# ProjectTorreyPines/TorJ.jl

Hardware: AMD Instinct MI355X
Metric: ray-steps/sec, 1e5-ray EC fan on 1 MI355X (+ 2/4/8-GPU scaling) (higher is better)
Workload: dtype f64

## Files before the change

torj.jl_amd/csrc/torj_args.hpp:

```cpp
#pragma once
#include "torj_math.hpp"

struct TraceArgs {
    const double *coef;
    const double *cellp;
    Grid g;
    Consts k;
    double omega;
    int mode;
    double ds;
    int n_steps;
    int chunk_steps;
    double psi_exit;
    double P_min;
    int n;
    const double *x0;
    const double *N0;
    const double *w;
    double *state;
    int *status;
    int *steps;
    int n_psi;
    const double *grid;
    double *dP;
// ... 36 lines not shown

struct SplitArgs {
    double *ain;
    double *alpha;
    unsigned *awork;
    double *psib;
    double *cbx;
    double *tx;
    int *tinfo;
    double *stau, *spsi, *sPdep;
    int *sinfo;
    unsigned char *zflag;
    double zval;
    int k0, kb;
    int nf;
    int tile_cap;
    double tile_margin;
    int traj_mode;
    int nan_step;
    unsigned long long *defer;
    unsigned *defer_cnt;
    int defer_lrm;
    int zlatch;
};

constexpr int kSplitMaxSteps = 1 << 24;
__device__ __forceinline__ int info_steps(int v) { return v & 0xffffff; }
__device__ __forceinline__ int info_status(int v) { return (unsigned)v >> 24; }
__device__ __forceinline__ int make_info(int steps, int st) { return steps | (st << 24); }

#ifndef TORJ_AIN_TRAJ_MATH
#define TORJ_AIN_TRAJ_MATH 0
#endif
#ifndef TORJ_TRAJ_WAVES
#define TORJ_TRAJ_WAVES TORJ_MIN_WAVES
#endif
#ifndef TORJ_ALPHA_WAVES
#define TORJ_ALPHA_WAVES 6
#endif
#ifndef TORJ_ALPHA_UNROLL
#define TORJ_ALPHA_UNROLL 1
#endif
#ifndef TORJ_TILE_NODES
#define TORJ_TILE_NODES 256
#endif
constexpr int kTileNodes = TORJ_TILE_NODES;
// ... 28 lines not shown
```

torj.jl_amd/csrc/torj_fitdepo.hpp:

```cpp
#pragma once
#include "torj_math.hpp"

namespace torj {

constexpr int kSmpBlk = 64;
TORJ_HD size_t smp_at(size_t j, int i, size_t rows) {
    return ((size_t)((unsigned)i / kSmpBlk) * rows + j) * kSmpBlk + (unsigned)i % kSmpBlk;
}
TORJ_HD size_t smp_elems(size_t n, size_t rows) { return (n + kSmpBlk - 1) / kSmpBlk * kSmpBlk * rows; }

struct FitArgs {
    const double *coef;
    Grid g;
    int n, n_psi;
    double ds;
    const double *grid;
    const double *w;
    const double *x_launch;
    const double *s0;
    const int *steps;
    const double *smp_psi, *smp_dpds, *smp_s;
    size_t rows;
    int s_uniform;
    double *E, *Gpsi, *GP;
    int *cnt;
    double *Fopen;
    double *dPs;
    int *kstar;
    double *dP;
    double *Pray;
    const int *npts;
};

TORJ_HD int imin(int x, int y) { return x < y ? x : y; }
TORJ_HD int imax(int x, int y) { return x > y ? x : y; }

constexpr int kChunk = 8;
constexpr int kWalkChunk = 4;
constexpr int kWalkChunkStream = 1;

struct RayData {
    const FitArgs *a;
    int i, m;
    double s0, psiL;
    TORJ_HD double S(int j) const {
        if (a->npts) return a->smp_s[smp_at(j, i, a->rows)];
        if (j == 0) return 0.0;
        return a->s_uniform ? fma((double)(j - 1), a->ds, s0) : a->smp_s[smp_at(j - 1, i, a->rows)];
    }
    TORJ_HD double h(int j) const { return (j == 0 && !a->npts) ? s0 : S(j + 1) - S(j); }
    TORJ_HD double Ypsi(int j) const {
        if (a->npts) return a->smp_psi[smp_at(j, i, a->rows)];
        return j == 0 ? psiL : a->smp_psi[smp_at(j - 1, i, a->rows)];
    }
// ... 553 lines not shown
```

torj.jl_amd/csrc/torj_hip.hip:

```cpp
#include <hip/hip_runtime.h>

#include <algorithm>
#include <cmath>
#include <cstring>
#include <mutex>
#include <vector>

#include "../../include/torj_hip.h"
#include "torj_math.hpp"
#include "torj_entry.hpp"
#include "torj_fitdepo.hpp"
#include "torj_warm.hpp"

using namespace torj;

#include "torj_host_util.hpp"
#include "torj_args.hpp"
#include "torj_k_fused.hpp"
#include "torj_k_traj.hpp"
#include "torj_k_alpha.hpp"
#include "torj_k_scan.hpp"
#include "torj_k_depo.hpp"
#include "torj_k_points.hpp"
#include "torj_k_beams.hpp"
// ... 136 lines not shown
        if (p->stage.h_pinned)
            (void)hipHostFree(p->stage.h);
        else
            free(p->stage.h);
    }
    for (int r = 0; r < 2; r++) {
        if (p->stage.up[r]) (void)hipEventDestroy(p->stage.up[r]);
        if (p->stage.tr[r]) (void)hipEventDestroy(p->stage.tr[r]);
        if (p->stage.dn[r]) (void)hipEventDestroy(p->stage.dn[r]);
    }
    if (p->stage.sc) (void)hipStreamDestroy(p->stage.sc);
    if (p->d_coef) (void)hipFree(p->d_coef);
    if (p->d_cellp) (void)hipFree(p->d_cellp);
    if (p->stream) (void)hipStreamDestroy(p->stream);
    if (p->ev_Nin) (void)hipEventDestroy(p->ev_Nin);
    if (p->ev_Nout) (void)hipEventDestroy(p->ev_Nout);
    if (p->sched.d) (void)hipFree(p->sched.d);
    if (p->fit.d) (void)hipFree(p->fit.d);
    if (p->d_flags) (void)hipFree(p->d_flags);
    if (p->chunk.d) (void)hipFree(p->chunk.d);
    for (hipEvent_t e : p->ev_pool) (void)hipEventDestroy(e);
    if (p->ws.d) (void)hipFree(p->ws.d);
    if (p->beams.d) (void)hipFree(p->beams.d);
    if (p->split.d) (void)hipFree(p->split.d);
    if (p->batch.d) (void)hipFree(p->batch.d);
    for (int q = 0; q < torj_plasma_s::kRing; q++) {
        if (p->ev_T[q]) (void)hipEventDestroy(p->ev_T[q]);
        if (p->ev_A[q]) (void)hipEventDestroy(p->ev_A[q]);
        if (p->ev_S[q]) (void)hipEventDestroy(p->ev_S[q]);
    }
    if (p->ev_J) (void)hipEventDestroy(p->ev_J);
    if (p->ev_F) (void)hipEventDestroy(p->ev_F);
    if (p->ev_D) (void)hipEventDestroy(p->ev_D);
    if (p->stream2) (void)hipStreamDestroy(p->stream2);
    if (p->streamT) (void)hipStreamDestroy(p->streamT);
    if (p->streamS) (void)hipStreamDestroy(p->streamS);
    if (p->streamD) (void)hipStreamDestroy(p->streamD);
    delete p;
    return 0;
}

int torj_plasma_get_coefs(torj_plasma_t p, int field, double *out) {
    if (!p || field < 0 || field > 5) return fail("bad plasma handle or field index");
    const size_t nodes = (size_t)(p->g.nR + 2) * (p->g.nZ + 2);
    for (size_t k = 0; k < nodes; k++) out[k] = p->coef[k * kNF + kFieldSlot[field]];
    return 0;
// ... 761 lines not shown
```

torj.jl_amd/csrc/torj_k_beams.hpp:

```cpp
#pragma once
#include "torj_args.hpp"
#include "torj_entry.hpp"
#include "torj_k_depo.hpp"
#include "torj_k_fused.hpp"
#include "torj_k_points.hpp"

__device__ __forceinline__ int beam_of(const BeamRec *beams, int n_beams, int i) {
    int lo = 0, hi = n_beams - 1;
    while (lo < hi) {
        const int mid = (lo + hi) >> 1;
        if (beams[mid].hi > i)
            hi = mid;
        else
            lo = mid + 1;
    }
    return lo;
}

__device__ __forceinline__ TraceArgs beam_args(const BeamsArgs &ba, int b, const BeamRec &br) {
    TraceArgs a = ba.a;
    a.omega = br.omega, a.k = br.k, a.mode = br.mode;
    if (a.dP) a.dP += (size_t)b * (size_t)(a.n_psi + 1);
    return a;
}

template <int ABS, int DEPO, bool TRAJ, int LPR = 1>
__global__ void __launch_bounds__(64, TORJ_MIN_WAVES) k_trace_beams(BeamsArgs ba) {
    const BeamWave wv = ba.waves[blockIdx.x];
    const BeamRec br = ba.beams[wv.beam];
    const TraceArgs a = beam_args(ba, wv.beam, br);
    const int i = wv.first + (int)threadIdx.x / LPR, sub = (int)threadIdx.x % LPR;
    AlbajarWork work = {};
    unsigned long long steps = 0;
    if (i < br.hi) {
        RayState r;
        load_start(a, i, r);
        const double w = (DEPO == kDepoBinned && a.w) ? a.w[i] : 1.0;
        ray_segment<ABS, DEPO, TRAJ, LPR>(a, i, w, r, a.n_steps, work, sub);
        if (sub == 0) {
            store_state(a, i, r);
// ... 2 lines not shown
        }
    }
    flush_counters(a, steps, 4ull * steps, work);
}

template <int ABS>
__global__ void __launch_bounds__(64) k_final_alpha_beams(BeamsArgs ba) {
    const TraceArgs &a = ba.a;
    const int i = blockIdx.x * 64 + threadIdx.x;
    if (i >= a.n) return;
    const int k = a.steps[i];
    if (k <= 0) return;
    const BeamRec br = ba.beams[beam_of(ba.beams, ba.n_beams, i)];
    double x[3], N[3], du[6], al = 0.0;
#pragma unroll
    for (int c = 0; c < 3; c++) {
        x[c] = a.state[c * a.n + i];
        N[c] = a.state[(3 + c) * a.n + i];
    }
    if constexpr (ABS != 0) ray_rhs_m<ABS>(a.coef, a.g, br.k, c_gl, br.omega, br.mode, a.abs_model, x, N, du, al, nullptr);
    a.smp_dpds[smp_at(k, i, a.smp_rows)] = exp(-a.state[6 * a.n + i]) * al;
}

__global__ void __launch_bounds__(256) k_shell_sum_beams(FitArgs a, const BeamRec *beams) {
    const int k = blockIdx.x;
    const int lo = beams[blockIdx.y].lo, nb = beams[blockIdx.y].hi - lo;
    double acc = 0.0;
    constexpr int kB = 8;
    const bool shell = k < a.n_psi - 1;
    const double *row = (shell ? a.dPs + (size_t)k * a.n : a.Pray) + lo;
    const double *wr = a.w ? a.w + lo : nullptr;
    const int *kstar = a.kstar + lo;
    for (int i0 = threadIdx.x; i0 < nb; i0 += 256 * kB) {
        double v[kB], wv[kB];
        bool on[kB];
#pragma unroll
        for (int u = 0; u < kB; u++) {
            const int i = i0 + 256 * u;
            on[u] = i < nb;
            v[u] = on[u] ? row[i] : 0.0;
            wv[u] = on[u] && wr ? wr[i] : 1.0;
            if (shell && on[u]) on[u] = k > kstar[i];
        }
#pragma unroll
        for (int u = 0; u < kB; u++)
            if (on[u]) acc += wv[u] * v[u];
    }
    __shared__ double red[4];
// ... 29 lines not shown
```

torj.jl_amd/csrc/torj_k_depo.hpp:

```cpp
#pragma once
#include "torj_args.hpp"
#include "torj_fitdepo.hpp"

constexpr int kFitGridLds = 4096;

__global__ void __launch_bounds__(64, 2) k_fit_depo(FitArgs a) {
    extern __shared__ double s_grid[];
    if (a.n_psi <= kFitGridLds) {
        for (int k = threadIdx.x; k < a.n_psi; k += 64) s_grid[k] = a.grid[k];
        __syncthreads();
        a.grid = s_grid;
    }
    const int i = blockIdx.x * 64 + threadIdx.x;
    if (i >= a.n) return;
    const double xl[3] = {a.x_launch[i], a.x_launch[a.n + i], a.x_launch[2 * a.n + i]};
    fit_depo_ray<kOpenCache>(a, i, psi_at(a.coef, a.g, xl));
}
__device__ __forceinline__ bool fit_grid_lds(FitArgs &a) {
    extern __shared__ double s_grid[];
    if (a.n_psi > kFitGridLds) return false;
    for (int k = threadIdx.x; k < a.n_psi; k += 64) s_grid[k] = a.grid[k];
    __syncthreads();
    a.grid = s_grid;
    return true;
}
__device__ __forceinline__ bool depo_stream_gate(const FitArgs &a, const DepoStream &ds, const int *sinfo,
                                                 int s_cap, int i, int &S, double &psiL) {
    const int v = __hip_atomic_load(sinfo + i, __ATOMIC_RELAXED, __HIP_MEMORY_SCOPE_AGENT);
    if (info_status(v) != ST_OK) return false;
    S = min(info_steps(v), s_cap);
    const int j = ds.v[kDsJ * (size_t)a.n + i];
    if ((j < 0 ? 0 : j) + kDepoQ + 3 + kDepoW > S) return false;
    psiL = 0.0;
    if (j < 0) {
        const double xl[3] = {a.x_launch[i], a.x_launch[a.n + i], a.x_launch[2 * a.n + i]};
        psiL = psi_at(a.coef, a.g, xl);
    }
    return true;
}
// ... 11 lines not shown
__global__ void __launch_bounds__(64, TORJ_DEPO_ELIM_WAVES) k_depo_elim(FitArgs a, DepoStream ds, const int *sinfo,
                                                                        int s_cap) {
    const int i = blockIdx.x * 64 + threadIdx.x;
    int S;
    double psiL;
    if (i >= a.n || !depo_stream_gate(a, ds, sinfo, s_cap, i, S, psiL)) return;
    fit_depo_stream_elim(a, ds, i, psiL, S);
}
#ifndef TORJ_DEPO_WALK_WAVES
#define TORJ_DEPO_WALK_WAVES 3
#endif
__global__ void __launch_bounds__(64, TORJ_DEPO_WALK_WAVES) k_depo_walk(FitArgs a, DepoStream ds, const int *sinfo,
                                                                        int s_cap) {
    fit_grid_lds(a);
    const int i = blockIdx.x * 64 + threadIdx.x;
    int S;
    double psiL;
    if (i >= a.n || !depo_stream_gate(a, ds, sinfo, s_cap, i, S, psiL)) return;
    fit_depo_stream_walk(a, ds, i, psiL, S);
}
__global__ void __launch_bounds__(64, 2) k_depo_tail(FitArgs a, DepoStream ds) {
    fit_grid_lds(a);
    const int i = blockIdx.x * 64 + threadIdx.x;
    if (i >= a.n) return;
    const double xl[3] = {a.x_launch[i], a.x_launch[a.n + i], a.x_launch[2 * a.n + i]};
    fit_depo_tail(a, ds, i, psi_at(a.coef, a.g, xl));
}
__global__ void __launch_bounds__(64) k_profile_samples(FitArgs a, const long *off, const double *s,
                                                        const double *x, size_t n_all, const double *dpds) {
    const int i = blockIdx.x * 64 + threadIdx.x;
    if (i >= a.n) return;
    for (int j = 0; j < a.npts[i]; j++) {
        const size_t q = (size_t)off[i] + j;
        const double xq[3] = {x[q], x[n_all + q], x[2 * n_all + q]};
        const size_t o = smp_at(j, i, a.rows);
        const_cast<double *>(a.smp_psi)[o] = psi_at(a.coef, a.g, xq);
        const_cast<double *>(a.smp_dpds)[o] = dpds[q];
        const_cast<double *>(a.smp_s)[o] = s[q];
    }
}
__global__ void __launch_bounds__(64, 2) k_fit_profile(FitArgs a) {
    extern __shared__ double s_grid[];
    if (a.n_psi <= kFitGridLds) {
        for (int k = threadIdx.x; k < a.n_psi; k += 64) s_grid[k] = a.grid[k];
        __syncthreads();
        a.grid = s_grid;
    }
    const int i = blockIdx.x * 64 + threadIdx.x;
    if (i >= a.n) return;
    fit_depo_ray<kOpenCache>(a, i, 0.0);
}
__global__ void __launch_bounds__(256) k_grid_check(const double *grid, int n, int *flags) {
    bool bad = false;
    for (int k = threadIdx.x + 1; k < n; k += 256) bad |= !(grid[k] > grid[k - 1]);
    if (bad) atomicOr(flags, 1);
}

__global__ void __launch_bounds__(256) k_shell_sum(FitArgs a) {
    const int k = blockIdx.x;
    double acc = 0.0;
    constexpr int kB = 8;
    const bool shell = k < a.n_psi - 1;
    const double *row = shell ? a.dPs + (size_t)k * a.n : a.Pray;
    for (int i0 = threadIdx.x; i0 < a.n; i0 += 256 * kB) {
        double v[kB], wv[kB];
        bool on[kB];
#pragma unroll
        for (int u = 0; u < kB; u++) {
            const int i = i0 + 256 * u;
            on[u] = i < a.n;
            v[u] = on[u] ? row[i] : 0.0;
            wv[u] = on[u] && a.w ? a.w[i] : 1.0;
            if (shell && on[u]) on[u] = k > a.kstar[i];
        }
#pragma unroll
        for (int u = 0; u < kB; u++)
            if (on[u]) acc += wv[u] * v[u];
    }
    __shared__ double red[4];
#pragma unroll
    for (int o = 32; o > 0; o >>= 1) acc += __shfl_xor(acc, o, 64);
    if ((threadIdx.x & 63) == 0) red[threadIdx.x >> 6] = acc;
// ... 8 lines not shown
```

torj.jl_amd/csrc/torj_k_scan.hpp:

```cpp
#pragma once
#include "torj_args.hpp"
#include "torj_k_fused.hpp"
#include "torj_k_traj.hpp"

__device__ void cold_replay(const TraceArgs &a, const SplitArgs &sp, int i, double x[3], double N[3], int k) {
    const TileCell cg{a.cellp, nullptr, 0, 0, 0, 0};
    const TileCoef ng{a.coef, nullptr, 0, 0, 0, 0};
    ZBox zb;
    for (int s = 0; s < k; s++) {
        double xn[3], Nn[3], psi;
        double *o_run = ain_row(a, sp, 0, i);
        if (sp.traj_mode == kTrajCell)
            cold_step<true, kTileNS, TileCell, true>(a, cg, sp, 0, i, x, N, xn, Nn, &psi, zb, false, o_run);
        else if (sp.traj_mode == kTrajTile)
            cold_step<true, kTileNS, TileCoef, true>(a, ng, sp, 0, i, x, N, xn, Nn, &psi, zb, false, o_run);
        else
            cold_step<true, kNF, const double *, true>(a, a.coef, sp, 0, i, x, N, xn, Nn, &psi, zb, false, o_run);
#pragma unroll
        for (int c = 0; c < 3; c++) {
            x[c] = xn[c];
            N[c] = Nn[c];
        }
    }
}
// ... 146 lines not shown
    double x[3], N[3];
    if (steps == tT && !(st & 0x40)) {
#pragma unroll
        for (int c = 0; c < 3; c++) {
            x[c] = sp.tx[c * (size_t)a.n + i];
            N[c] = sp.tx[(3 + c) * (size_t)a.n + i];
        }
    } else {
        const int cs = a.chunk_steps > 0 ? a.chunk_steps : 1 << 30;
        const int c0 = a.chunk_steps > 0 ? steps / cs : 0;
        const double *cb = sp.cbx + (size_t)c0 * 6 * a.n + i;
#pragma unroll
        for (int c = 0; c < 3; c++) {
            x[c] = cb[c * (size_t)a.n];
            N[c] = cb[(3 + c) * (size_t)a.n];
        }
        cold_replay(a, sp, i, x, N, steps - c0 * (a.chunk_steps > 0 ? cs : 0));
        if constexpr (TRAJ) {
            if (a.traj_stride > 0)
                for (int k = steps / a.traj_stride; k < min(tT, a.n_steps) / a.traj_stride; k++)
                    for (int r = 0; r < 5; r++) a.traj[((size_t)k * 5 + r) * a.n + i] = NAN;
        }
    }
    st &= 0x3f;
#pragma unroll
    for (int c = 0; c < 3; c++) {
        a.state[c * a.n + i] = x[c];
        a.state[(3 + c) * a.n + i] = N[c];
    }
    a.state[6 * a.n + i] = sp.stau[i];
    a.status[i] = st;
    a.steps[i] = steps;
    const double Pdep = sp.sPdep[i];
    if (a.Pdep) a.Pdep[i] = Pdep;
    if constexpr (DEPO == kDepoBinned) {
        const double w = a.w ? a.w[i] : 1.0;
        atomicAdd(a.dP + a.n_psi, w * Pdep);
    }
}
```

torj.jl_amd/csrc/torj_k_traj.hpp:

```cpp
#pragma once
#include "torj_args.hpp"
#include "torj_fitdepo.hpp"


#ifndef TORJ_TRAJ_AIN_STEP
#define TORJ_TRAJ_AIN_STEP 1
#endif
__device__ __forceinline__ double *ain_row(const TraceArgs &a, const SplitArgs &sp, int row, int i) {
    return sp.ain + ((size_t)row * sp.nf) * a.n + i;
}
template <bool STORE, int NS = kNF, class CS = const double *, bool PSI = false>
__device__ __forceinline__ bool cold_step(const TraceArgs &a, CS coef,
                                          const SplitArgs &sp, int j, int i, const double x[3],
                                          const double N[3], double xn[3], double Nn[3],
                                          double *psi_x, ZBox &zb, bool zon, double *&o_run) {
    const double hds = 0.5 * a.ds, ds6 = a.ds / 6.0;
    double acc[6] = {0, 0, 0, 0, 0, 0}, xt[3], Nt[3], k[6];
#pragma unroll
    for (int c = 0; c < 3; c++) {
        xt[c] = x[c];
        Nt[c] = N[c];
    }
    constexpr bool kCellTrim = IsTileCell<CS>::value;
#pragma unroll 1
// ... 175 lines not shown
        sp.tx[c * (size_t)a.n + i] = x[c];
        sp.tx[(3 + c) * (size_t)a.n + i] = N[c];
    }
    sp.tinfo[i] = make_info(steps, st);
    if (sp.zflag != nullptr) sp.zflag[i] = zero_box_flag(zb) ? 1 : 0;
}


template <int DEPO, bool TRAJ, int MODE>
__device__ __forceinline__ void traj_body(const TraceArgs &a, const SplitArgs &sp) {
    const int i = blockIdx.x * blockDim.x + threadIdx.x;
    double x[3] = {0, 0, 0}, N[3] = {0, 0, 0};
    int steps = 0, st = ST_OK;
    bool live = i < a.n;
    if (live) {
        if (sp.k0 == 0) {
#pragma unroll
            for (int c = 0; c < 3; c++) {
                x[c] = a.x0[c * a.n + i];
                N[c] = a.N0[c * a.n + i];
                sp.cbx[c * (size_t)a.n + i] = x[c];
                sp.cbx[(3 + c) * (size_t)a.n + i] = N[c];
            }
        } else {
            const int v = sp.tinfo[i];
            steps = info_steps(v);
            st = info_status(v);
#pragma unroll
            for (int c = 0; c < 3; c++) {
                x[c] = sp.tx[c * (size_t)a.n + i];
                N[c] = sp.tx[(3 + c) * (size_t)a.n + i];
            }
        }
        live = st == ST_OK && !(sp.k0 > 0 && info_status(sp.sinfo[i]) != ST_OK);
        if (!live && sp.zflag) sp.zflag[i] = 1;
    }
    if constexpr (MODE == kTrajTile) {
        __shared__ __attribute__((aligned(16))) double s_tile[kTileNodes * kTileNS];
        const double R = sqrt(x[0] * x[0] + x[1] * x[1]);
        const double inf = __builtin_inf();
        const double rmin = wave_min(live ? R : inf), rmax = wave_max(live ? R : -inf);
        const double zmin = wave_min(live ? x[2] : inf), zmax = wave_max(live ? x[2] : -inf);
        if (!(rmin <= rmax && zmin <= zmax)) return;
        const double m = (double)(sp.kb + 1) * a.ds * sp.tile_margin;
        const int iR0 = cell_index(rmin - m, a.g.R1, a.g.Rn, a.g.invhR, a.g.nR),
                  iR1 = cell_index(rmax + m, a.g.R1, a.g.Rn, a.g.invhR, a.g.nR),
// ... 90 lines not shown
```

torj.jl_amd/csrc/torj_launch.hpp:

```cpp
#pragma once
#include <algorithm>
#include <cmath>
#include <vector>

#include "../../include/torj_hip.h"
#include "torj_args.hpp"
#include "torj_fitdepo.hpp"
#include "torj_host_util.hpp"

enum FitArr { kFaPsi, kFaDpds, kFaS, kFaE, kFaGpsi, kFaGP, kFaCnt, kFaFopen, kFaDPs, kFaKstar, kFaN };

static size_t fit_arr_bytes(int k, size_t rows, size_t n_psi, bool store_s) {
    if (k <= kFaGP) return k == kFaS && !store_s ? 0 : sizeof(double) * rows;
    return k == kFaCnt ? sizeof(int) * (n_psi + 1) : k == kFaKstar ? sizeof(int) : sizeof(double) * n_psi;
}

static size_t fit_bytes_per_ray(size_t rows, size_t n_psi, bool store_s) {
    size_t b = 0;
    for (int k = 0; k < kFaN; k++) b += fit_arr_bytes(k, rows, n_psi, store_s);
    return b;
}

struct FitLayout {
    size_t rows;
// ... 219 lines not shown
    with_abs_depo_traj(a.abs_model, pl.DM, pl.tr, [&](auto A, auto D, auto Tr) {
        constexpr bool T = A() >= 2 || Tr();
        if (pl.adaptive)
            hipLaunchKernelGGL((k_trace_sched<A(), D(), T, 1>), grd, blk, pl.lds, s, a, ctl, slots, pl.S, pl.G, pl.cs);
        else
            hipLaunchKernelGGL((k_trace_sched<A(), D(), T, 0>), grd, blk, pl.lds, s, a, ctl, slots, pl.S, pl.G, pl.cs);
    });
    hipLaunchKernelGGL(k_sched_fold, dim3(1), dim3(1), 0, s, ctl, (unsigned)pl.G, p->d_flags);
    return 0;
}

static void launch_lanes(const TraceArgs &a, const LaunchPlan &pl, hipStream_t s) {
    const dim3 grd(pl.grid), blk(TORJ_BLOCK);
    if (pl.path == kPathLane16)
        with_depo_traj(pl.DM, pl.tr, [&](auto D, auto T) {
            if constexpr (D() != kDepoBinned) hipLaunchKernelGGL((k_trace<1, D(), T(), 16>), grd, blk, 0, s, a);
        });
    else
        with_abs_depo_traj(a.abs_model == 1 ? 1 : 0, pl.DM, pl.tr, [&](auto A, auto D, auto T) {
            if constexpr (A() <= 1) hipLaunchKernelGGL((k_trace<A(), D(), T()>), grd, blk, 0, s, a);
        });
}

static int launch_post(const TraceArgs &a, const FitArgs &fa, const LaunchPlan &pl, const DepoStream &dstr,
                       hipStream_t s) {
    const dim3 grd(nblocks(a.n, 64)), blk(64);
    if (!pl.adaptive)
        with_abs(a.abs_model, [&](auto A) { hipLaunchKernelGGL(k_final_alpha<A()>, grd, blk, 0, s, a); });
    const size_t lds = fit_grid_lds(fa.n_psi);
    if (dstr.v)
        hipLaunchKernelGGL(k_depo_tail, grd, blk, lds, s, fa, dstr);
    else
        hipLaunchKernelGGL(k_fit_depo, grd, blk, lds, s, fa);
    hipLaunchKernelGGL(k_shell_sum, dim3(fa.n_psi), dim3(256), 0, s, fa);
    HIPCK(hipGetLastError());
    return 0;
}

static int timing_begin(torj_plasma_s *p, hipEvent_t ev[3], hipStream_t s) {
    ev[0] = ev[1] = ev[2] = nullptr;
    if (!p->timing) return 0;
    while (p->ev_used + 3 > p->ev_pool.size()) {
        hipEvent_t e;
        HIPCK(hipEventCreate(&e));
        p->ev_pool.push_back(e);
    }
    for (int q = 0; q < 3; q++) ev[q] = p->ev_pool[p->ev_used + q];
    p->ev_used += 3;
    HIPCK(hipEventRecord(ev[0], s));
    return 0;
}

static TraceArgs trace_args(const torj_plasma_s *p, const torj_trace_cfg &cfg, int n, const double *x0,
                            const double *N0, const double *weights, const double *s0, double *state,
                            int *status, int *steps, uint64_t *counters) {
    TraceArgs a{};
    a.coef = p->d_coef, a.cellp = p->d_cellp, a.g = p->g;
// ... 31 lines not shown
    if (fresh && launch_plan(pl, *cfg, n, n_psi, has, launch_knobs(p))) return -1;
    if (cfg->absorption == 1 && ensure_gl_on_device(p->device)) return -1;
    hipStream_t s = (hipStream_t)stream;
    TraceArgs a = trace_args(p, *cfg, n, x0, N0, weights, s0, state, status, steps, counters);
    if (pl.adaptive) {
        if (ensure_buf(p, p->chunk, (size_t)n * sizeof(int))) return -1;
        a.chunk = (int *)p->chunk.d;
    }
    if (pl.depo) {
        a.n_psi = n_psi;
        a.grid = grid;
        a.dP = dP;
        if (!Pdep) {
            if (ensure_buf(p, p->ws, (size_t)n * sizeof(double))) return -1;
            Pdep = (double *)p->ws.d;
        }
        a.Pdep = Pdep;
    }
    FitArgs fa{};
    if (pl.fit) {
        if (ensure_buf(p, p->fit, pl.lay.bytes())) return -1;
        fit_point(pl.lay, (char *)p->fit.d, fa, &a);
        fit_args(fa, a, x_launch, !pl.adaptive);
    }
    if (pl.depo)
        hipLaunchKernelGGL(k_grid_check, dim3(1), dim3(256), 0, s, grid, n_psi, p->d_flags);
    if (pl.tr) {
        a.traj_stride = cfg->traj_stride, a.n_save = pl.n_save, a.traj = traj;
        if (a.n_save > 0)
            HIPCK(hipMemsetAsync(traj, 0xFF, (size_t)a.n_save * 5 * n * sizeof(double), s));
    }
    if (pl.fit && pl.path != kPathSplit && fit_zero(fa, s)) return -1;
    hipEvent_t ev[3];
    if (timing_begin(p, ev, s)) return -1;
    DepoStream dstr{};
    switch (pl.path) {
    case kPathSplit:
        if (split_trace(p, a, pl.DM, pl.tr, s, pl.fit ? &fa : nullptr, &dstr, g_gl_host.negl_skip != 0)) return -1;
        break;
    case kPathQueue:
        if (launch_queue(p, a, pl, s)) return -1;
        break;
    case kPathLane1:
    case kPathLane16: launch_lanes(a, pl, s);
    }
    HIPCK(hipGetLastError());
    if (ev[1]) HIPCK(hipEventRecord(ev[1], s));
    if (pl.fit && launch_post(a, fa, pl, dstr, s)) return -1;
    if (ev[2]) HIPCK(hipEventRecord(ev[2], s));
    return 0;
}

// ... 42 lines not shown
            return fail("multi-beam launch: the reference deposition's workspace for %d rays (%zu bytes) exceeds "
                        "the budget of %zu bytes (TORJ_WS_GB); trace the beams in separate calls",
                        n, bp.lay.bytes(), budget);
    }
    BeamsArgs ba{};
    torj_trace_cfg c1 = *cfg;
    c1.omega = omega[0], c1.mode = mode[0];
    TraceArgs &a = ba.a = trace_args(p, c1, n, x0, N0, weights, s0, state, status, steps, counters);
    ba.n_beams = n_beams;
    if (beams_upload(p, bp.beams, bp.waves, s, &ba.beams, &ba.waves)) return -1;
    if (bp.depo) {
        a.n_psi = n_psi, a.grid = grid, a.dP = dP;
        if (!Pdep) {
            if (ensure_buf(p, p->ws, (size_t)n * sizeof(double))) return -1;
            Pdep = (double *)p->ws.d;
        }
        a.Pdep = Pdep;
    }
    FitArgs fa{};
    if (bp.fit) {
        if (ensure_buf(p, p->fit, bp.lay.bytes())) return -1;
        fit_point(bp.lay, (char *)p->fit.d, fa, &a);
        fit_args(fa, a, x_launch, true);
    }
    if (bp.depo) hipLaunchKernelGGL(k_grid_check, dim3(1), dim3(256), 0, s, grid, n_psi, p->d_flags);
    if (bp.tr) {
        a.traj_stride = cfg->traj_stride, a.n_save = bp.n_save, a.traj = traj;
        if (a.n_save > 0)
            HIPCK(hipMemsetAsync(traj, 0xFF, (size_t)a.n_save * 5 * n * sizeof(double), s));
    }
    if (bp.fit && fit_zero(fa, s)) return -1;
    hipEvent_t ev[3];
    if (timing_begin(p, ev, s)) return -1;
    launch_beams(ba, bp, s);
    HIPCK(hipGetLastError());
    if (ev[1]) HIPCK(hipEventRecord(ev[1], s));
    if (bp.fit) {
        const dim3 grd(nblocks(n, 64)), blk(64);
        with_abs(a.abs_model, [&](auto A) {
            if constexpr (A() <= 1) hipLaunchKernelGGL(k_final_alpha_beams<A()>, grd, blk, 0, s, ba);
        });
        hipLaunchKernelGGL(k_fit_depo, grd, blk, fit_grid_lds(fa.n_psi), s, fa);
        hipLaunchKernelGGL(k_shell_sum_beams, dim3(fa.n_psi, n_beams), dim3(256), 0, s, fa, ba.beams);
        HIPCK(hipGetLastError());
    }
    if (ev[2]) HIPCK(hipEventRecord(ev[2], s));
    return 0;
}

static int trace_batched(torj_plasma_t p, const torj_trace_cfg *cfg, int n, int nb, const double *x0,
                         const double *N0, const double *weights, int n_psi, const double *grid,
                         const double *x_launch, const double *s0, double *state, int *status, int *steps,
                         double *dP, double *Pdep, double *traj, uint64_t *counters, hipStream_t s) {
    const int n_save = cfg->traj_stride > 0 && traj ? cfg->n_steps / cfg->traj_stride : 0;
    const size_t D = sizeof(double), B = (size_t)nb;
    enum { kX0, kN0, kXl, kW, kS0, kP, kSt, kTr, kNb };
    const int rows[kNb] = {3, 3, 3, 1, 1, 1, 7, 5 * n_save};
    size_t off[kNb + 1] = {0};
    for (int k = 0; k < kNb; k++) off[k + 1] = off[k] + (size_t)rows[k];
    if (ensure_buf(p, p->batch, off[kNb] * B * D + 2 * B * sizeof(int))) return -1;
    auto b = [&](int k) { return (double *)p->batch.d + off[k] * B; };
    int *bstat = (int *)b(kNb), *bsteps = bstat + B;
    for (int lo = 0; lo < n; lo += nb) {
        const int c = std::min(nb, n - lo);
        auto gather = [&](int k, const double *h) -> int {
            if (!h) return 0;
// ... 22 lines not shown
```

torj.jl_amd/csrc/torj_math.hpp:

```cpp
#pragma once

#include <hip/hip_runtime.h>
#include <math.h>
#include <stdint.h>

#include "torj_bessel_coefs.hpp"

#define TORJ_HD __host__ __device__ __forceinline__

namespace torj {

constexpr double kC = 2.99792458e8;
constexpr double kE = 1.602176634e-19;
constexpr double kMe = 9.1093837015e-31;
constexpr double kEps0 = 8.8541878128e-12;
constexpr double kPi = 3.14159265358979323846;

constexpr int kNF = 8;
enum Field { F_BR = 0, F_BPHI = 1, F_BZ = 2, F_LNNE = 3, F_LNTE = 4, F_PSI = 5 };

enum Status { ST_OK = 0, ST_LEFT_PLASMA = 1, ST_ABSORBED = 2, ST_NAN = 3, ST_REFLECTED = 4,
              ST_ENTRY_FAIL = 5, ST_MAX_STEPS = 6 };

struct Grid {
// ... 152 lines not shown
TORJ_HD void axis_setup(double x, double x1, double xn, double invh, int n, Axis &a) {
    const double xc = clampd(x, x1, xn);
    a.delta = x - xc;
    const double u = (xc - x1) * invh;
    int i = (int)floor(u);
    i = i < 0 ? 0 : (i > n - 2 ? n - 2 : i);
    bweights(u - (double)i, a.w, a.dw);
    a.i = i;
}

template <int NGRAD, int NVAL>
struct FieldPack {
    static constexpr int NG1 = NGRAD > 0 ? NGRAD : 1;
    double v[NGRAD + NVAL];
    double dR[NG1], dZ[NG1];
};

struct alignas(16) Dbl2 {
    double x, y;
};
template <class P>
struct Pair16Ptr {
    using type = const Dbl2 *;
};
#ifdef __HIP_DEVICE_COMPILE__
template <>
struct Pair16Ptr<const __attribute__((address_space(3))) double *> {
    using type = const __attribute__((address_space(3))) Dbl2 *;
};
template <>
struct Pair16Ptr<const __attribute__((address_space(1))) double *> {
    using type = const __attribute__((address_space(1))) Dbl2 *;
};
#endif

template <int NGRAD, int NVAL, bool EXT, int NS, class P = const double *>
TORJ_HD void stencil_sums(P c0, int rs, const Axis &aR, const Axis &aZ,
                          const int (&fidx)[NGRAD + NVAL], double (&v)[NGRAD + NVAL],
                          double (&gr)[NGRAD + NVAL], double (&gz)[NGRAD + NVAL],
                          double (&grz)[NGRAD + NVAL]) {
    constexpr int NT = NGRAD + NVAL;
#pragma unroll
    for (int f = 0; f < NT; f++) v[f] = gr[f] = gz[f] = grz[f] = 0.0;
    auto field = [&](int f, int b, const double (&c)[4]) {
        const bool slopes = EXT || f < NGRAD;
        double sv = 0.0, sd = 0.0;
#pragma unroll
        for (int a = 0; a < 4; a++) {
            sv = fma(aR.w[a], c[a], sv);
            if (slopes) sd = fma(aR.dw[a], c[a], sd);
        }
        v[f] = fma(aZ.w[b], sv, v[f]);
        if (slopes) {
            gz[f] = fma(aZ.dw[b], sv, gz[f]);
            gr[f] = fma(aZ.w[b], sd, gr[f]);
// ... 163 lines not shown
    asm("v_max_f64 %0, %1, %2" : "=v"(xc) : "v"(x), "s"(x1));
    asm("v_min_f64 %0, %1, %2" : "=v"(xc) : "v"(xc), "s"(xn));
    a.delta = x - xc;
    const double u = (xc - x1) * invh;
    int i;
    asm("v_med3_i32 %0, %1, 0, %2" : "=v"(i) : "v"((int)u), "s"(n - 2));
    a.t = (u - (double)i) * h;
    a.i = i;
#else
    const double xc = clampd(x, x1, xn);
    a.delta = x - xc;
    const double u = (xc - x1) * invh;
    int i = (int)floor(u);
    i = i < 0 ? 0 : (i > n - 2 ? n - 2 : i);
    a.t = (u - (double)i) * h;
    a.i = i;
#endif
}
struct TileCell {
    const double *g;
    const double *lds;
    int cR0, cZ0, cw, ch;
};
TORJ_HD void cell_field(const Dbl2 (&A)[8], double tR, double tZ, bool SLOPES, bool CROSS, double &v,
                        double &gr, double &gz, double &grz) {
    double p[4], d[4];
#pragma unroll
    for (int j = 0; j < 4; j++) {
        const Dbl2 lo = A[2 * j], hi = A[2 * j + 1];
        const double p1 = fma(hi.y, tR, hi.x);
        const double p2 = fma(p1, tR, lo.y);
        p[j] = fma(p2, tR, lo.x);
        if (SLOPES) d[j] = fma(fma(hi.y, tR, p1), tR, p2);
    }
    const double q1 = fma(p[3], tZ, p[2]);
    const double q2 = fma(q1, tZ, p[1]);
    v = fma(q2, tZ, p[0]);
    if (SLOPES) {
        gz = fma(fma(p[3], tZ, q1), tZ, q2);
        const double r1 = fma(d[3], tZ, d[2]);
        const double r2 = fma(r1, tZ, d[1]);
        gr = fma(r2, tZ, d[0]);
        if (CROSS) grz = fma(fma(d[3], tZ, r1), tZ, r2);
    }
}
template <int NGRAD, int NVAL, bool EXT, class P>
TORJ_HD void cell_sums(P c, const CellAxis &aR, const CellAxis &aZ, const int (&fidx)[NGRAD + NVAL],
                       double (&v)[NGRAD + NVAL], double (&gr)[NGRAD + NVAL], double (&gz)[NGRAD + NVAL],
                       double (&grz)[NGRAD + NVAL]) {
    constexpr int NT = NGRAD + NVAL;
    const double tR = aR.t, tZ = aZ.t;
    using Q = typename Pair16Ptr<P>::type;
#pragma unroll
    for (int f = 0; f < NT; f++) {
        Dbl2 A[8];
#pragma unroll
        for (int k = 0; k < 8; k++) A[k] = reinterpret_cast<Q>(c + fidx[f] * 16)[k];
        cell_field(A, tR, tZ, EXT || f < NGRAD, EXT && f < NGRAD, v[f], gr[f], gz[f], grz[f]);
    }
}
template <int NGRAD, int NVAL, bool EXT = true, int NS = kNF>
TORJ_HD void eval_fields(const TileCell &t, const Grid &g, const CellAxis &aR, const CellAxis &aZ,
                         const int (&fidx)[NGRAD + NVAL], FieldPack<NGRAD, NVAL> &out) {
    constexpr int NT = NGRAD + NVAL;
    const int dR = aR.i - t.cR0, dZ = aZ.i - t.cZ0;
    bool in = kCellAxisFast ? (unsigned)dR < (unsigned)t.cw && (unsigned)dZ < (unsigned)t.ch
                            : dR >= 0 && dR < t.cw && dZ >= 0 && dZ < t.ch;
#ifdef __HIP_DEVICE_COMPILE__
    in = __all(in);
    using LdsP = const __attribute__((address_space(3))) double *;
    using GlbP = const __attribute__((address_space(1))) double *;
#else
    using LdsP = const double *;
    using GlbP = const double *;
#endif
// ... 942 lines not shown
```

torj.jl_amd/csrc/torj_plasma.hpp:

```cpp
#pragma once
#include <rccl/rccl.h>

#include <algorithm>
#include <mutex>
#include <vector>

#include "torj_host_util.hpp"
#include "torj_math.hpp"

static void bspl1d_prefilter(int n, const double *y, size_t ystride, double *c, size_t cstride) {
    auto C = [&](int k) -> double & { return c[(size_t)k * cstride]; };
    auto Y = [&](int k) { return y[(size_t)k * ystride]; };
    C(1) = Y(0);
    C(n) = Y(n - 1);
    const int m = n - 2;
    if (m > 0) {
        std::vector<double> cp(m), dp(m);
        for (int k = 0; k < m; k++) {
            double r = 6.0 * Y(k + 1);
            if (k == 0) r -= C(1);
            if (k == m - 1) r -= C(n);
            const double den = 4.0 - (k > 0 ? cp[k - 1] : 0.0);
            cp[k] = 1.0 / den;
            dp[k] = (r - (k > 0 ? dp[k - 1] : 0.0)) / den;
// ... 81 lines not shown
struct torj_plasma_s {
    int device = 0;
    Grid g{};
    std::vector<double> coef;
    double *d_coef = nullptr;
    double *d_cellp = nullptr;
    int n_vol = 0;
    double v1 = 0, vn = 0;
    std::vector<double> vol_coef;
    double psi_prof_max = 0;
    hipStream_t stream = nullptr;
    GrowBuf sched;
    int sched_mode = -1, sched_waves = 0;
    int lanes_per_ray = 0;
    GrowBuf chunk;
    GrowBuf fit;
    bool timing = false;
    int timing_calls = 0;
    GrowBuf batch;
    std::vector<hipEvent_t> ev_pool;
    size_t ev_used = 0;
    GrowBuf ws;
    GrowBuf beams;
    int *d_flags = nullptr;
    int n_cu = 256;
    std::mutex mu;
    std::vector<torj_plasma_s *> replicas;
    std::vector<ncclComm_t> comms;
    struct BeamStage {
        void *d = nullptr, *h = nullptr;
        size_t d_cap = 0, h_cap = 0;
        bool h_pinned = false;
        hipStream_t sc = nullptr;
        hipEvent_t up[2] = {}, tr[2] = {}, dn[2] = {};
    } stage;
    double reduce_ms = 0.0;
    int reduce_calls = 0;
    GrowBuf split;
    hipStream_t stream2 = nullptr, streamT = nullptr;
    hipStream_t streamS = nullptr;
    hipStream_t streamD = nullptr;
    static constexpr int kRing = 4;
    hipEvent_t ev_T[kRing] = {}, ev_A[kRing] = {}, ev_S[kRing] = {}, ev_J = nullptr, ev_F = nullptr;
    hipEvent_t ev_D = nullptr;
    hipEvent_t ev_Nin = nullptr, ev_Nout = nullptr;
};
// ... 130 lines not shown
```

torj.jl_amd/csrc/torj_split.hpp:

```cpp
#pragma once
#include <atomic>

#include "torj_dispatch.hpp"
#include "torj_k_alpha.hpp"
#include "torj_k_depo.hpp"
#include "torj_k_scan.hpp"
#include "torj_k_traj.hpp"
#include "torj_plasma.hpp"

static size_t fit_grid_lds(int n_psi) { return n_psi <= kFitGridLds ? (size_t)n_psi * sizeof(double) : 0; }

static int fit_zero(const FitArgs &fa, hipStream_t st) {
    const size_t L = (size_t)fa.n_psi, N = (size_t)fa.n;
    HIPCK(hipMemsetAsync(fa.cnt, 0, (L + 1) * N * sizeof(int), st));
    HIPCK(hipMemsetAsync(fa.Fopen, 0xFF, L * N * sizeof(double), st));
    HIPCK(hipMemsetAsync(fa.dPs, 0, L * N * sizeof(double), st));
    return 0;
}

struct SplitPlan {
    static constexpr int R = torj_plasma_s::kRing;
    size_t n;
    int n_steps, nf;
    long kb, first;
    int n_blk;
    size_t b_ain, b_alpha, b_awork, b_psib, b_cbx, b_n8, b_n4, b_zf, b_dsd, b_dsi, b_defer, b_dcnt, bytes;
    bool zflag_on, dstream, serial;
    int dstream_env, depo_lag, lds_env, tile_cap, nan_step, zflag_nan_from, defer_lrm, zlatch;
    double tile_margin;

    int block_k0(int b) const { return (int)(first ? (b == 0 ? 0 : first + (long)(b - 1) * kb) : b * kb); }
    int block_len(int b) const { return (int)std::min<long>(first && b == 0 ? first : kb, n_steps - block_k0(b)); }
    int window_cap(int bw) const {
        return (int)(first ? (bw == 0 ? first : first + (long)bw * kb) : std::min<long>((long)(bw + 1) * kb, n_steps));
    }
};
// ... 121 lines not shown
    sp.nan_step = pl.nan_step;
    sp.zval = 0.0;
    sp.defer_lrm = pl.defer_lrm;
    sp.zlatch = pl.zlatch;

    const bool serial = pl.serial, dstream = pl.dstream;
    static const bool scan_own = env_int("TORJ_SPLIT_SCAN", 1) != 0;
    hipStream_t sT = serial ? s : p->streamT, s2 = serial ? s : p->stream2;
    hipStream_t s3 = serial ? s : (scan_own ? p->streamS : p->stream2);
    const bool depo_own = dstream && (pl.dstream_env == 2 || pl.dstream_env == 4) && !serial;
    const bool depo_traj = dstream && pl.dstream_env == 5 && !serial;
    if (depo_own && !p->streamD) {
        int lo = 0, hi = 0;
        HIPCK(hipDeviceGetStreamPriorityRange(&lo, &hi));
        HIPCK(hipStreamCreateWithPriority(&p->streamD, hipStreamNonBlocking, stream_prio("TORJ_DEPO_PRIO", lo, lo, hi)));
    }
    hipStream_t sD = depo_own ? p->streamD : s3;
    if (!serial) {
        HIPCK(hipEventRecord(p->ev_F, s));
        HIPCK(hipStreamWaitEvent(sT, p->ev_F, 0));
        HIPCK(hipStreamWaitEvent(s2, p->ev_F, 0));
        if (s3 != s2) HIPCK(hipStreamWaitEvent(s3, p->ev_F, 0));
    }
    HIPCK(hipMemsetAsync(sp.stau, 0, 3 * pl.b_n8, sT));
    HIPCK(hipMemsetAsync(sp.sinfo, 0, pl.b_n4, sT));
    if (dstream) HIPCK(hipMemsetAsync(ds.v + kDsJ * n, 0xFF, n * sizeof(int), sT));
    if (rg.dcnt) HIPCK(hipMemsetAsync(rg.dcnt, 0, pl.n_blk * sizeof(unsigned), s2));
    if (fa && fit_zero(*fa, s3)) return -1;
    const size_t fit_lds = fa ? fit_grid_lds(fa->n_psi) : 0;
    const int G = (int)((n + 63) / 64);
    const size_t lds_bytes = (size_t)(a.g.nR + 2) * (a.g.nZ + 2) * kTrajLdsNS * sizeof(double);
    const bool lds_traj = pl.lds_env == 1 && lds_bytes <= 160 * 1024;
    const bool tile_traj = pl.lds_env == 2, cell_traj = pl.lds_env == 3;
    sp.traj_mode = cell_traj ? kTrajCell : tile_traj ? kTrajTile : lds_traj ? kTrajLds : kTrajL2;
    const int wpb = std::min(8, std::max(1, (G + p->n_cu - 1) / p->n_cu));
    const int n_blocks = pl.n_blk;
    auto depo_pair = [&](hipStream_t st, int cap) {
        hipLaunchKernelGGL(k_depo_elim, dim3(G), dim3(64), 0, st, *fa, ds, sp.sinfo, cap);
        hipLaunchKernelGGL(k_depo_walk, dim3(G), dim3(64), fit_lds, st, *fa, ds, sp.sinfo, cap);
    };
    for (int b = 0; b < n_blocks; b++) {
        sp.k0 = pl.block_k0(b);
        sp.kb = pl.block_len(b);
        const int r = b % R;
        sp.ain = rg.ain[r];
        sp.psib = rg.psib[r];
        sp.zflag = rg.zflags[r];
        sp.zval = (pl.zflag_nan_from >= 0 && sp.k0 >= pl.zflag_nan_from) ? NAN : 0.0;
        sp.alpha = rg.alphas[r];
// ... 91 lines not shown
```

Measured before the change: 5.831 billion.

## Skip inner shell sums below min kstar, fold split memsets into kernels, pipeline cell loads

Adds a device-wide (or per-beam) minimum of kstar via wave reductions and atomicMin, and uses it to let shell-sum blocks at or below that index exit early. Moves the split path's stau/spsi/sPdep/sinfo/dsj zeroing and the trajectory NaN fill into the trace and scan kernels in place of separate memsets. Adds a software-pipelined LDS variant of cell_sums that loads the next field's coefficients while evaluating the current one, separated by a sched barrier. These changes aim to cut launch and memset overhead and idle shell-sum work, at the cost of extra atomics, an extra memset for kmin, and correctness that depends on the skip condition holding.

After: 5.858 billion, median of 6. Within noise of the previous version (+0.5%).

```diff
diff --git a/torj.jl_amd/csrc/torj_args.hpp b/torj.jl_amd/csrc/torj_args.hpp
--- a/torj.jl_amd/csrc/torj_args.hpp
+++ b/torj.jl_amd/csrc/torj_args.hpp
@@ -82,6 +82,7 @@
     unsigned *defer_cnt;
     int defer_lrm;
     int zlatch;
+    int *dsj;
 };
 
 constexpr int kSplitMaxSteps = 1 << 24;
diff --git a/torj.jl_amd/csrc/torj_fitdepo.hpp b/torj.jl_amd/csrc/torj_fitdepo.hpp
--- a/torj.jl_amd/csrc/torj_fitdepo.hpp
+++ b/torj.jl_amd/csrc/torj_fitdepo.hpp
@@ -30,6 +30,7 @@
     double *dP;
     double *Pray;
     const int *npts;
+    int *kmin;
 };
 
 TORJ_HD int imin(int x, int y) { return x < y ? x : y; }
diff --git a/torj.jl_amd/csrc/torj_hip.hip b/torj.jl_amd/csrc/torj_hip.hip
--- a/torj.jl_amd/csrc/torj_hip.hip
+++ b/torj.jl_amd/csrc/torj_hip.hip
@@ -182,6 +182,7 @@
     for (hipEvent_t e : p->ev_pool) (void)hipEventDestroy(e);
     if (p->ws.d) (void)hipFree(p->ws.d);
     if (p->beams.d) (void)hipFree(p->beams.d);
+    if (p->kmin.d) (void)hipFree(p->kmin.d);
     if (p->split.d) (void)hipFree(p->split.d);
     if (p->batch.d) (void)hipFree(p->batch.d);
     for (int q = 0; q < torj_plasma_s::kRing; q++) {
diff --git a/torj.jl_amd/csrc/torj_k_beams.hpp b/torj.jl_amd/csrc/torj_k_beams.hpp
--- a/torj.jl_amd/csrc/torj_k_beams.hpp
+++ b/torj.jl_amd/csrc/torj_k_beams.hpp
@@ -5,17 +5,6 @@
 #include "torj_k_fused.hpp"
 #include "torj_k_points.hpp"
 
-__device__ __forceinline__ int beam_of(const BeamRec *beams, int n_beams, int i) {
-    int lo = 0, hi = n_beams - 1;
-    while (lo < hi) {
-        const int mid = (lo + hi) >> 1;
-        if (beams[mid].hi > i)
-            hi = mid;
-        else
-            lo = mid + 1;
-    }
-    return lo;
-}
 
 __device__ __forceinline__ TraceArgs beam_args(const BeamsArgs &ba, int b, const BeamRec &br) {
     TraceArgs a = ba.a;
@@ -64,8 +53,9 @@
     a.smp_dpds[smp_at(k, i, a.smp_rows)] = exp(-a.state[6 * a.n + i]) * al;
 }
 
-__global__ void __launch_bounds__(256) k_shell_sum_beams(FitArgs a, const BeamRec *beams) {
+__global__ void __launch_bounds__(256) k_shell_sum_beams(FitArgs a, const BeamRec *beams, const int *kmin) {
     const int k = blockIdx.x;
+    if (kmin && k < a.n_psi - 1 && k <= kmin[blockIdx.y]) return;
     const int lo = beams[blockIdx.y].lo, nb = beams[blockIdx.y].hi - lo;
     double acc = 0.0;
     constexpr int kB = 8;
diff --git a/torj.jl_amd/csrc/torj_k_depo.hpp b/torj.jl_amd/csrc/torj_k_depo.hpp
--- a/torj.jl_amd/csrc/torj_k_depo.hpp
+++ b/torj.jl_amd/csrc/torj_k_depo.hpp
@@ -4,7 +4,25 @@
 
 constexpr int kFitGridLds = 4096;
 
-__global__ void __launch_bounds__(64, 2) k_fit_depo(FitArgs a) {
+__device__ __forceinline__ int beam_of(const BeamRec *beams, int n_beams, int i) {
+    int lo = 0, hi = n_beams - 1;
+    while (lo < hi) {
+        const int mid = (lo + hi) >> 1;
+        if (beams[mid].hi > i)
+            hi = mid;
+        else
+            lo = mid + 1;
+    }
+    return lo;
+}
+__device__ __forceinline__ void kstar_min_wave(const FitArgs &a, int ks) {
+    if (!a.kmin) return;
+#pragma unroll
+    for (int o = 32; o > 0; o >>= 1) ks = min(ks, __shfl_xor(ks, o, 64));
+    if (threadIdx.x == 0) atomicMin(a.kmin, ks);
+}
+
+__global__ void __launch_bounds__(64, 2) k_fit_depo(FitArgs a, const BeamRec *beams, int n_beams) {
     extern __shared__ double s_grid[];
     if (a.n_psi <= kFitGridLds) {
         for (int k = threadIdx.x; k < a.n_psi; k += 64) s_grid[k] = a.grid[k];
@@ -12,9 +30,14 @@
         a.grid = s_grid;
     }
     const int i = blockIdx.x * 64 + threadIdx.x;
-    if (i >= a.n) return;
-    const double xl[3] = {a.x_launch[i], a.x_launch[a.n + i], a.x_launch[2 * a.n + i]};
-    fit_depo_ray<kOpenCache>(a, i, psi_at(a.coef, a.g, xl));
+    int ks = 0x7fffffff;
+    if (i < a.n) {
+        const double xl[3] = {a.x_launch[i], a.x_launch[a.n + i], a.x_launch[2 * a.n + i]};
+        fit_depo_ray<kOpenCache>(a, i, psi_at(a.coef, a.g, xl));
+        ks = a.kstar[i];
+        if (beams && a.kmin) atomicMin(a.kmin + beam_of(beams, n_beams, i), ks);
+    }
+    if (!beams) kstar_min_wave(a, ks);
 }
 __device__ __forceinline__ bool fit_grid_lds(FitArgs &a) {
     extern __shared__ double s_grid[];
@@ -72,9 +95,13 @@
 __global__ void __launch_bounds__(64, 2) k_depo_tail(FitArgs a, DepoStream ds) {
     fit_grid_lds(a);
     const int i = blockIdx.x * 64 + threadIdx.x;
-    if (i >= a.n) return;
-    const double xl[3] = {a.x_launch[i], a.x_launch[a.n + i], a.x_launch[2 * a.n + i]};
-    fit_depo_tail(a, ds, i, psi_at(a.coef, a.g, xl));
+    int ks = 0x7fffffff;
+    if (i < a.n) {
+        const double xl[3] = {a.x_launch[i], a.x_launch[a.n + i], a.x_launch[2 * a.n + i]};
+        fit_depo_tail(a, ds, i, psi_at(a.coef, a.g, xl));
+        ks = a.kstar[i];
+    }
+    kstar_min_wave(a, ks);
 }
 __global__ void __launch_bounds__(64) k_profile_samples(FitArgs a, const long *off, const double *s,
                                                         const double *x, size_t n_all, const double *dpds) {
@@ -106,8 +133,9 @@
     if (bad) atomicOr(flags, 1);
 }
 
-__global__ void __launch_bounds__(256) k_shell_sum(FitArgs a) {
+__global__ void __launch_bounds__(256) k_shell_sum(FitArgs a, const int *kmin) {
     const int k = blockIdx.x;
+    if (kmin && k < a.n_psi - 1 && k <= *kmin) return;
     double acc = 0.0;
     constexpr int kB = 8;
     const bool shell = k < a.n_psi - 1;
diff --git a/torj.jl_amd/csrc/torj_k_scan.hpp b/torj.jl_amd/csrc/torj_k_scan.hpp
--- a/torj.jl_amd/csrc/torj_k_scan.hpp
+++ b/torj.jl_amd/csrc/torj_k_scan.hpp
@@ -192,6 +192,11 @@
                     for (int r = 0; r < 5; r++) a.traj[((size_t)k * 5 + r) * a.n + i] = NAN;
         }
     }
+    if constexpr (TRAJ) {
+        if (a.traj_stride > 0)
+            for (int k = min(tT, a.n_steps) / a.traj_stride; k < a.n_save; k++)
+                for (int r = 0; r < 5; r++) a.traj[((size_t)k * 5 + r) * a.n + i] = __longlong_as_double(-1ll);
+    }
     st &= 0x3f;
 #pragma unroll
     for (int c = 0; c < 3; c++) {
diff --git a/torj.jl_amd/csrc/torj_k_traj.hpp b/torj.jl_amd/csrc/torj_k_traj.hpp
--- a/torj.jl_amd/csrc/torj_k_traj.hpp
+++ b/torj.jl_amd/csrc/torj_k_traj.hpp
@@ -221,6 +221,11 @@
                 sp.cbx[c * (size_t)a.n + i] = x[c];
                 sp.cbx[(3 + c) * (size_t)a.n + i] = N[c];
             }
+            sp.stau[i] = 0.0;
+            sp.spsi[i] = 0.0;
+            sp.sPdep[i] = 0.0;
+            sp.sinfo[i] = 0;
+            if (sp.dsj) sp.dsj[i] = -1;
         } else {
             const int v = sp.tinfo[i];
             steps = info_steps(v);
diff --git a/torj.jl_amd/csrc/torj_launch.hpp b/torj.jl_amd/csrc/torj_launch.hpp
--- a/torj.jl_amd/csrc/torj_launch.hpp
+++ b/torj.jl_amd/csrc/torj_launch.hpp
@@ -265,6 +265,10 @@
         });
 }
 
+static const int *shell_skip_word(const FitArgs &fa) {
+    return env_int("TORJ_SHELL_SKIP", 1) != 0 ? fa.kmin : nullptr;
+}
+
 static int launch_post(const TraceArgs &a, const FitArgs &fa, const LaunchPlan &pl, const DepoStream &dstr,
                        hipStream_t s) {
     const dim3 grd(nblocks(a.n, 64)), blk(64);
@@ -274,8 +278,8 @@
     if (dstr.v)
         hipLaunchKernelGGL(k_depo_tail, grd, blk, lds, s, fa, dstr);
     else
-        hipLaunchKernelGGL(k_fit_depo, grd, blk, lds, s, fa);
-    hipLaunchKernelGGL(k_shell_sum, dim3(fa.n_psi), dim3(256), 0, s, fa);
+        hipLaunchKernelGGL(k_fit_depo, grd, blk, lds, s, fa, (const BeamRec *)nullptr, 0);
+    hipLaunchKernelGGL(k_shell_sum, dim3(fa.n_psi), dim3(256), 0, s, fa, shell_skip_word(fa));
     HIPCK(hipGetLastError());
     return 0;
 }
@@ -353,12 +357,14 @@
         if (ensure_buf(p, p->fit, pl.lay.bytes())) return -1;
         fit_point(pl.lay, (char *)p->fit.d, fa, &a);
         fit_args(fa, a, x_launch, !pl.adaptive);
+        if (ensure_buf(p, p->kmin, kMaxBeams * sizeof(int))) return -1;
+        fa.kmin = (int *)p->kmin.d;
     }
     if (pl.depo)
         hipLaunchKernelGGL(k_grid_check, dim3(1), dim3(256), 0, s, grid, n_psi, p->d_flags);
     if (pl.tr) {
         a.traj_stride = cfg->traj_stride, a.n_save = pl.n_save, a.traj = traj;
-        if (a.n_save > 0)
+        if (a.n_save > 0 && pl.path != kPathSplit)
             HIPCK(hipMemsetAsync(traj, 0xFF, (size_t)a.n_save * 5 * n * sizeof(double), s));
     }
     if (pl.fit && pl.path != kPathSplit && fit_zero(fa, s)) return -1;
@@ -447,6 +453,8 @@
         if (ensure_buf(p, p->fit, bp.lay.bytes())) return -1;
         fit_point(bp.lay, (char *)p->fit.d, fa, &a);
         fit_args(fa, a, x_launch, true);
+        if (ensure_buf(p, p->kmin, kMaxBeams * sizeof(int))) return -1;
+        fa.kmin = (int *)p->kmin.d;
     }
     if (bp.depo) hipLaunchKernelGGL(k_grid_check, dim3(1), dim3(256), 0, s, grid, n_psi, p->d_flags);
     if (bp.tr) {
@@ -454,7 +462,7 @@
         if (a.n_save > 0)
             HIPCK(hipMemsetAsync(traj, 0xFF, (size_t)a.n_save * 5 * n * sizeof(double), s));
     }
-    if (bp.fit && fit_zero(fa, s)) return -1;
+    if (bp.fit && fit_zero(fa, s, n_beams)) return -1;
     hipEvent_t ev[3];
     if (timing_begin(p, ev, s)) return -1;
     launch_beams(ba, bp, s);
@@ -465,8 +473,9 @@
         with_abs(a.abs_model, [&](auto A) {
             if constexpr (A() <= 1) hipLaunchKernelGGL(k_final_alpha_beams<A()>, grd, blk, 0, s, ba);
         });
-        hipLaunchKernelGGL(k_fit_depo, grd, blk, fit_grid_lds(fa.n_psi), s, fa);
-        hipLaunchKernelGGL(k_shell_sum_beams, dim3(fa.n_psi, n_beams), dim3(256), 0, s, fa, ba.beams);
+        hipLaunchKernelGGL(k_fit_depo, grd, blk, fit_grid_lds(fa.n_psi), s, fa, ba.beams, n_beams);
+        hipLaunchKernelGGL(k_shell_sum_beams, dim3(fa.n_psi, n_beams), dim3(256), 0, s, fa, ba.beams,
+                           shell_skip_word(fa));
         HIPCK(hipGetLastError());
     }
     if (ev[2]) HIPCK(hipEventRecord(ev[2], s));
diff --git a/torj.jl_amd/csrc/torj_math.hpp b/torj.jl_amd/csrc/torj_math.hpp
--- a/torj.jl_amd/csrc/torj_math.hpp
+++ b/torj.jl_amd/csrc/torj_math.hpp
@@ -198,15 +198,18 @@
 template <class P>
 struct Pair16Ptr {
     using type = const Dbl2 *;
+    static constexpr bool lds = false;
 };
 #ifdef __HIP_DEVICE_COMPILE__
 template <>
 struct Pair16Ptr<const __attribute__((address_space(3))) double *> {
     using type = const __attribute__((address_space(3))) Dbl2 *;
+    static constexpr bool lds = true;
 };
 template <>
 struct Pair16Ptr<const __attribute__((address_space(1))) double *> {
     using type = const __attribute__((address_space(1))) Dbl2 *;
+    static constexpr bool lds = false;
 };
 #endif
 
@@ -416,17 +419,23 @@
     const double *lds;
     int cR0, cZ0, cw, ch;
 };
+TORJ_HD void cell_row(const Dbl2 lo, const Dbl2 hi, double tR, bool SLOPES, double &p, double &d) {
+    const double p1 = fma(hi.y, tR, hi.x);
+    const double p2 = fma(p1, tR, lo.y);
+    p = fma(p2, tR, lo.x);
+    if (SLOPES) d = fma(fma(hi.y, tR, p1), tR, p2);
+}
+TORJ_HD void cell_cols(const double (&p)[4], const double (&d)[4], double tZ, bool SLOPES, bool CROSS, double &v,
+                       double &gr, double &gz, double &grz);
 TORJ_HD void cell_field(const Dbl2 (&A)[8], double tR, double tZ, bool SLOPES, bool CROSS, double &v,
                         double &gr, double &gz, double &grz) {
     double p[4], d[4];
 #pragma unroll
-    for (int j = 0; j < 4; j++) {
-        const Dbl2 lo = A[2 * j], hi = A[2 * j + 1];
-        const double p1 = fma(hi.y, tR, hi.x);
-        const double p2 = fma(p1, tR, lo.y);
-        p[j] = fma(p2, tR, lo.x);
-        if (SLOPES) d[j] = fma(fma(hi.y, tR, p1), tR, p2);
-    }
+    for (int j = 0; j < 4; j++) cell_row(A[2 * j], A[2 * j + 1], tR, SLOPES, p[j], d[j]);
+    cell_cols(p, d, tZ, SLOPES, CROSS, v, gr, gz, grz);
+}
+TORJ_HD void cell_cols(const double (&p)[4], const double (&d)[4], double tZ, bool SLOPES, bool CROSS, double &v,
+                       double &gr, double &gz, double &grz) {
     const double q1 = fma(p[3], tZ, p[2]);
     const double q2 = fma(q1, tZ, p[1]);
     v = fma(q2, tZ, p[0]);
@@ -438,6 +447,12 @@
         if (CROSS) grz = fma(fma(d[3], tZ, r1), tZ, r2);
     }
 }
+#ifndef TORJ_CELL_PIPE
+#define TORJ_CELL_PIPE 1
+#endif
+#ifndef TORJ_CELL_PIPE_FENCE
+#define TORJ_CELL_PIPE_FENCE() __builtin_amdgcn_sched_barrier(0x2)
+#endif
 template <int NGRAD, int NVAL, bool EXT, class P>
 TORJ_HD void cell_sums(P c, const CellAxis &aR, const CellAxis &aZ, const int (&fidx)[NGRAD + NVAL],
                        double (&v)[NGRAD + NVAL], double (&gr)[NGRAD + NVAL], double (&gz)[NGRAD + NVAL],
@@ -445,6 +460,47 @@
     constexpr int NT = NGRAD + NVAL;
     const double tR = aR.t, tZ = aZ.t;
     using Q = typename Pair16Ptr<P>::type;
+#if TORJ_CELL_PIPE && defined(__HIP_DEVICE_COMPILE__)
+  if constexpr (Pair16Ptr<P>::lds) {
+    Dbl2 A[8];
+#pragma unroll
+    for (int k = 0; k < 8; k++) A[k] = reinterpret_cast<Q>(c + fidx[0] * 16)[k];
+#pragma unroll
+    for (int f = 0; f < NT; f++) {
+        const bool SLOPES = EXT || f < NGRAD, CROSS = EXT && f < NGRAD;
+        double pj = 0.0, dj = 0.0, q = 0.0, tq = 0.0, r = 0.0, tr = 0.0;
+#pragma unroll
+        for (int j = 3; j >= 0; j--) {
+            const double pu = pj, du = dj;
+            cell_row(A[2 * j], A[2 * j + 1], tR, SLOPES, pj, dj);
+            if (j == 2) {
+                q = fma(pu, tZ, pj);
+                if (SLOPES) {
+                    tq = fma(pu, tZ, q);
+                    r = fma(du, tZ, dj);
+                    if (CROSS) tr = fma(du, tZ, r);
+                }
+            } else if (j == 1) {
+                q = fma(q, tZ, pj);
+                if (SLOPES) {
+                    gz[f] = fma(tq, tZ, q);
+                    r = fma(r, tZ, dj);
+                    if (CROSS) grz[f] = fma(tr, tZ, r);
+                }
+            } else if (j == 0) {
+                v[f] = fma(q, tZ, pj);
+                if (SLOPES) gr[f] = fma(r, tZ, dj);
+            }
+            if (f + 1 < NT) {
+                A[2 * j] = reinterpret_cast<Q>(c + fidx[f + 1] * 16)[2 * j];
+                A[2 * j + 1] = reinterpret_cast<Q>(c + fidx[f + 1] * 16)[2 * j + 1];
+                TORJ_CELL_PIPE_FENCE();
+            }
+        }
+    }
+    return;
+  }
+#endif
 #pragma unroll
     for (int f = 0; f < NT; f++) {
         Dbl2 A[8];
diff --git a/torj.jl_amd/csrc/torj_plasma.hpp b/torj.jl_amd/csrc/torj_plasma.hpp
--- a/torj.jl_amd/csrc/torj_plasma.hpp
+++ b/torj.jl_amd/csrc/torj_plasma.hpp
@@ -127,6 +127,7 @@
     size_t ev_used = 0;
     GrowBuf ws;
     GrowBuf beams;
+    GrowBuf kmin;
     int *d_flags = nullptr;
     int n_cu = 256;
     std::mutex mu;
diff --git a/torj.jl_amd/csrc/torj_split.hpp b/torj.jl_amd/csrc/torj_split.hpp
--- a/torj.jl_amd/csrc/torj_split.hpp
+++ b/torj.jl_amd/csrc/torj_split.hpp
@@ -10,8 +10,9 @@
 
 static size_t fit_grid_lds(int n_psi) { return n_psi <= kFitGridLds ? (size_t)n_psi * sizeof(double) : 0; }
 
-static int fit_zero(const FitArgs &fa, hipStream_t st) {
+static int fit_zero(const FitArgs &fa, hipStream_t st, int n_kmin = 1) {
     const size_t L = (size_t)fa.n_psi, N = (size_t)fa.n;
+    if (fa.kmin) HIPCK(hipMemsetAsync(fa.kmin, 0x7F, (size_t)n_kmin * sizeof(int), st));
     HIPCK(hipMemsetAsync(fa.cnt, 0, (L + 1) * N * sizeof(int), st));
     HIPCK(hipMemsetAsync(fa.Fopen, 0xFF, L * N * sizeof(double), st));
     HIPCK(hipMemsetAsync(fa.dPs, 0, L * N * sizeof(double), st));
@@ -179,9 +180,7 @@
         HIPCK(hipStreamWaitEvent(s2, p->ev_F, 0));
         if (s3 != s2) HIPCK(hipStreamWaitEvent(s3, p->ev_F, 0));
     }
-    HIPCK(hipMemsetAsync(sp.stau, 0, 3 * pl.b_n8, sT));
-    HIPCK(hipMemsetAsync(sp.sinfo, 0, pl.b_n4, sT));
-    if (dstream) HIPCK(hipMemsetAsync(ds.v + kDsJ * n, 0xFF, n * sizeof(int), sT));
+    sp.dsj = dstream ? ds.v + kDsJ * n : nullptr;
     if (rg.dcnt) HIPCK(hipMemsetAsync(rg.dcnt, 0, pl.n_blk * sizeof(unsigned), s2));
     if (fa && fit_zero(*fa, s3)) return -1;
     const size_t fit_lds = fa ? fit_grid_lds(fa->n_psi) : 0;
```
